# mhrice/RemFx

Hardware: AMD Instinct MI355X
Metric: audio-seconds/sec fwd+bwd (whole job) (higher is better)
Workload: dtype bf16 (fp32 accumulate); 1 GPU; Hybrid Demucs (cfg/model/demucs.yaml) train step, +exp=chorus_aug model=demucs; clips_per_gpu=64, global_batch=64, clip_samples=262144, parallelism=dp1, rccl_ranks=0, ranks=1, streams=4

## Files before the change

### include/remfx_hip.h

```cpp
#ifndef REMFX_HIP_H
#define REMFX_HIP_H

#include <stdint.h>

#ifdef __cplusplus
extern "C" {
#endif

#define RFX_ABI_VERSION 1

enum rfx_act {
  RFX_ACT_NONE = 0,
  RFX_ACT_RELU = 1,
  RFX_ACT_GELU = 2,
  RFX_ACT_TANH = 3,
  RFX_ACT_PRELU = 4,
  RFX_ACT_LEAKY = 5,
  RFX_ACT_SIGMOID = 6
};

typedef struct rfx_ktab_entry {
  int32_t off;
  int32_t da;
  int32_t db;
// ... 255 lines not shown
                       const float* sums, float w_sc, float w_lm, const float* gup, float* gxc, void* stream);
int64_t rfx_stft_pair_loss_ws(const rfx_stft_desc* d);
int rfx_stft_pair_loss(const rfx_stft_desc* d, const float* x, const float* y, const float* window, float eps, double* ws, float* sums,
                       float* xspec, float* ymag, void* stream);
int rfx_stft_loss_grad_m(const float* xc, const float* ymag, int32_t R, int64_t n, float eps, const float* sums, float w_sc,
                         float w_lm, const float* gup, float* gxc, void* stream);
int rfx_fft_synthesis_lossgrad(const rfx_stft_desc* d, const float* xspec, const float* ymag, const float* sums, float w_sc,
                               float w_lm, float eps, const float* gup, const float* window, float* ws, float* out, void* stream);
int rfx_l1_grad(const float* a, const float* b, int64_t n, float w, const float* gup, float* g, void* stream);
#define RFX_SISDR_SLOTS 128
int rfx_sisdr_sums(const float* x, const float* t, int32_t R, int64_t L, int64_t x_rs, int64_t t_rs,
                   double* ws, double* sums, void* stream);
int rfx_sisdr_finish(const double* sums, int32_t R, int64_t L, int32_t zero_mean, double eps, float* out, void* stream);
int rfx_mrstft_combine(const float* const* sums, const int64_t* n, int32_t nres, int32_t R, int32_t per_example_sc, float* out,
                       void* stream);

int rfx_zero(void* p, int64_t nbytes, void* stream);
#define RFX_SUMSQ_SLOTS 4096
int rfx_sumsq(const float* g, int64_t n, double* ws, double* out, void* stream);
int rfx_clip_coef(const double* sumsq, float max_norm, float pre, float* coef, float* norm_out, void* stream);
int rfx_adamw_step(float* p, const float* g, float* m, float* v, int64_t n, float lr, float b1, float b2,
                   float eps, float wd, int32_t step, const float* gscale, void* stream);

typedef struct rfx_cl_tensor {
  void* p;
  int64_t ns, as;
  int32_t bs, c0;
} rfx_cl_tensor;

enum rfx_cl_epi {
  RFX_CL_STORE = 0,
  RFX_CL_GELU = 1,
  RFX_CL_GLU = 2,
  RFX_CL_DGELU = 3,
  RFX_CL_STORE_CM = 5,
  RFX_CL_DGLU = 4
};

typedef struct rfx_cl_conv_desc {
  rfx_cl_tensor in;
  int32_t N, IA, IB, OA, OB, SA;
  int32_t NTR, NCH, NTC, KS;
  int32_t da0, da_step;
  int32_t db0, db_step;
  int32_t wrapb;
  const void* apack;
  int32_t M, BM;
  int32_t mode;
  int32_t G, g_off, OAo, Co;
  const float* bias;
  const float* rowadd;
  rfx_cl_tensor out0, out1, aux0, res;
  void* cm_out;
  int64_t cm_ns, cm_cs, cm_as;
  int32_t cm_fold;
} rfx_cl_conv_desc;
int rfx_cl_conv(const rfx_cl_conv_desc* d, void* stream);
int rfx_cl_pack(const float* src, const int32_t* idx, int64_t n, void* dst, void* stream);
int rfx_cl_from_cm(const void* src, int32_t src_bf16, int64_t s_ns, int64_t s_cs, int64_t s_as, int32_t N, int32_t C, int32_t A,
                   int32_t B, const rfx_cl_tensor* dst, const rfx_cl_tensor* res, const rfx_cl_tensor* aux, int32_t mode, void* stream);
int rfx_cl_to_cm(const rfx_cl_tensor* src, int32_t N, int32_t C, int32_t A, int32_t B, void* dst, int32_t dst_bf16, int64_t d_ns,
                 int64_t d_cs, int64_t d_as, const void* aux16, void* stream);
int rfx_cl_im2col_s4(const float* src, int64_t s_ns, int64_t s_cs, int64_t s_as, int32_t N, int32_t Cs, int32_t IA, int32_t IB, int32_t OA,
                     int32_t OB, int32_t along_b, void* dst, void* stream);
int rfx_cl_im2col_fm(const float* src, const float* coef_a, const float* coef_b, int32_t N, int32_t F, int32_t bins, void* dst, void* stream);
int rfx_fm_cm_affine(const float* in, float* out, const float* coef_a, const float* coef_b, int32_t N, int32_t bins, int32_t F, int32_t to_fm,
                     void* stream);
int rfx_cl_dgelu(const void* g, const void* z, void* out, int64_t n, void* stream);
int rfx_cl_dglu(const void* g, const void* zab, void* out, int64_t npos, int32_t C, void* stream);

typedef struct rfx_cl_wgrad_desc {
  rfx_cl_tensor p, q;
  int32_t N, OA, IA, B;
  int32_t SA, da0, NTR;
  int32_t NTC, db0, db_step;
  int32_t M, Cq, CW;
  int32_t RW, WK;
  int32_t S, ahead, bias;
  int32_t PW;
  float* ws;
} rfx_cl_wgrad_desc;
int64_t rfx_cl_wgrad_ws_floats(const rfx_cl_wgrad_desc* d);
int rfx_cl_wgrad(const rfx_cl_wgrad_desc* d, void* stream);
int rfx_cl_wgrad_reduce(const float* ws, const int32_t* map, int64_t nmap, int32_t S, int32_t DT, int32_t RW, int32_t WK, float* dw,
                        int64_t wn, float* db, int32_t accumulate, void* stream);

typedef struct rfx_cl_dconv_desc {
  const void* x;
  const void* gy;
  void* y;
  void* a; void* hpre; float* stats;
  void* dz; void* dh; float* partial;
  const void* w1p; const void* w2p; const void* w2dp; const void* w1dp;
  const float *b1, *g1w, *g1b, *b2, *g2w, *g2b, *scale;
  int32_t S, C, H, dil, grid, x_or_gy_ok;
  float eps;
  int32_t TPS;
  float* tsum; float* sums;
  float* pg_dst[5];
} rfx_cl_dconv_desc;
int rfx_cl_dconv_ok(int32_t C, int32_t H, int32_t T, int32_t backward);
int rfx_cl_dconv_fwd(const rfx_cl_dconv_desc* d, void* stream);
int rfx_cl_dconv_bwd(const rfx_cl_dconv_desc* d, float* pgrad, void* stream);

int rfx_cl_rowsum(const rfx_cl_tensor* x, int32_t N, int32_t A, int32_t B, int32_t C, int32_t G, float scale, float* partial, float* out,
                  int32_t accumulate, void* stream);

int rfx_abi_version(void);
int rfx_gemm_pick_r(int32_t M, int32_t K);

#ifdef __cplusplus
}
#endif
#endif
```

### remfx_amd/_lib.py

```python
import ctypes as C
import glob
import os
import subprocess

_HERE = os.path.dirname(os.path.abspath(__file__))
_ROOT = os.path.dirname(_HERE)
CSRC = os.path.join(_HERE, "csrc")
INCLUDE = os.path.join(_ROOT, "include")
LIBDIR = os.path.join(_HERE, "_C")
LIBPATH = os.environ.get("RFX_LIBPATH_DEV") or os.path.join(LIBDIR, "libremfx_hip.so")

HIPCC_FLAGS = ["--offload-arch=gfx950", "-O3", "-std=c++17", "-fPIC", "-ffp-contract=fast",
               "-I" + INCLUDE, "-I" + CSRC]


def sources():
    return sorted(glob.glob(os.path.join(CSRC, "*.hip")))


def _stale():
    if not os.path.exists(LIBPATH):
        return True
    t = os.path.getmtime(LIBPATH)
    deps = sources() + glob.glob(os.path.join(CSRC, "*.h")) + glob.glob(os.path.join(INCLUDE, "*.h"))
# ... 118 lines not shown
    "rfx_norm_bwd_work_floats": [_I32, _I32, _I32, _I32],
    "rfx_batchnorm_stat_slots": [_I32, _I32],
    "rfx_groupnorm_fwd": [_P, _P, _P, _I32, _I32, _I32, _I32, C.c_float, _I32, _P, _P, _P, _I32, _P, _P, _P, _P],
    "rfx_groupnorm_bwd": [_P, _P, _P, _P, _P, _P, _I32, _I32, _I32, _I32, _I32, _P, _P, _P, _P, _P, _P, _P],
    "rfx_groupnorm_fwd_x16": [_P, _P, _P, _I32, _I32, _I32, _I32, C.c_float, _I32, _P, _P, _P, _I32, _P, _P, _P, _P],
    "rfx_groupnorm_bwd_x16": [_P, _P, _P, _P, _P, _P, _I32, _I32, _I32, _I32, _I32, _P, _P, _P, _P, _P, _P, _P],
    "rfx_batchnorm_fwd": [_P, _P, _P, _I32, _I32, _I32, C.c_float, _I32, _I32, _P, _P, _P, _P, _P],
    "rfx_batchnorm_bwd": [_P, _P, _P, _P, _P, _P, _I32, _I32, _I32, _I32, _P, _P, _P, _P, _P],
    "rfx_avgpool2d_fwd": [_P, _P, _I64, _I32, _I32, _I32, _I32, _P],
    "rfx_avgpool2d_bwd": [_P, _P, _I64, _I32, _I32, _I32, _I32, _P],
    "rfx_cplx_slots": [_I32, _I64],
    "rfx_cplx_moments": [_P, _I32, _I32, _I64, _P, _P, _P],
    "rfx_cplx_moments_bwd": [_P, _P, _I32, _I32, _I64, _P, _P],
    "rfx_cplx_coef_fwd": [_P, C.c_double, _P, _P, _P, _P, _P, _P, C.c_float, _I32, _P, _P, _P, _P, _P, _P, _P, C.c_float, _P],
    "rfx_cplx_coef_bwd": [_P, C.c_double, _P, _P, _P, _P, _P, _P, C.c_float, _I32, _P, _P, _P, _P],
    "rfx_cplx_affine_act_fwd": [_P, _P, _I32, _I32, _I64, C.c_float, _P, _I64, _I64, _P],
    "rfx_cplx_affine_act_bwd": [_P, _P, _P, _I64, _I64, _I32, _I32, _I64, C.c_float, _P, _P, _P, _P],
    "rfx_bound_mask_fwd": [_P, _P, _P, _I32, _I64, _I64, _I64, _I64, _P],
    "rfx_bound_mask_bwd": [_P, _P, _P, _P, _I32, _I64, _I64, _I64, _I64, _I64, _P],
    "rfx_phase_mask_fwd": [_P, _P, _P, _I64, _P],
    "rfx_phase_mask_bwd": [_P, _P, _P, _I64, _P],
    "rfx_glu_fwd": [_P, _P, _I64, _I64, _I64, _P],
    "rfx_glu_bwd": [_P, _P, _P, _I64, _I64, _I64, _P],
    "rfx_glu_bwd_bf16": [_P, _P, _P, _I64, _I64, _I64, _P],
    "rfx_act_fwd": [_P, _P, _I64, _I32, _P],
    "rfx_act_bwd": [_P, _P, _P, _I64, _I32, _P],
    "rfx_act_add_fwd": [_P, _P, _P, _I64, _I32, _P],
    "rfx_act_rows": [_P, _I64, _I64, _I64, _P, _I64, _I64, _I64, _P, _I64, _I64, _I64, _I32, _I32, _I32, _I32, _I32, _P],
    "rfx_act_rows16": [_P, _I64, _I64, _I64, _P, _I64, _I64, _I64, _P, _I64, _I64, _I64, _I32, _I32, _I32, _I32, _I32, _P],
    "rfx_mul": [_P, _P, _P, _I64, _P],
    "rfx_prelu_fwd": [_P, _P, _P, _I64, _I64, _I64, _P],
    "rfx_prelu_bwd": [_P, _P, _P, _P, _P, _P, _I64, _I64, _I64, _P],
    "rfx_l1_sum": [_P, _P, _I64, _P, C.c_float, _P, _P],
    "rfx_add_bcast": [_P, _P, _P, _I64, _I32, _I32, _I32, _I64, _I64, _I64, _I64, C.c_float, _P],
    "rfx_localstate_fwd": [_P, _P, _P, _P, _I32, _I32, _I32, _I32, _I32, _P, _P, _P],
    "rfx_localstate_bwd": [_P, _P, _P, _P, _P, _P, _I32, _I32, _I32, _I32, _I32, _P, _P, _P, _P, _P],
    "rfx_dconv_layer_ok": [_I32, _I32, _I32],
    "rfx_dconv_layer_bwd_rows": [_I32],
    "rfx_dconv_layer_bwd": [_P, _P, _P, _I32, _I32, _I32, _I32, _P, _P, _P, _P, _P, _P, _P, _P, _P, C.c_float, _P, _P, _P, _P, _P],
    "rfx_dconv_layer_fwd": [_P, _P, _I32, _I32, _I32, _I32, _P, _P, _P, _P, _P, _P, _P, _P, _P, C.c_float, _P, _P, _P, _P, _P],
    "rfx_fx_distortion": [_P, _P, _I32, _I64, _P, _P],
    "rfx_fx_delay": [_P, _P, _I32, _I64, _P, _P, _P, _P],
    "rfx_fx_chorus": [_P, _P, _I32, _I64, C.c_float, _P, _P, _P, _P, _P, _P],
    "rfx_fx_compressor": [_P, _P, _P, _I32, _I64, _P, _P, _P, _P, _P],
    "rfx_fx_reverb": [_P, _P, _I32, _I64, _I32, _P, _P, _P, _P, _P],
    "rfx_fx_loudness": [_P, _I32, _I64, _I32, _I32, _I32, _I32, C.c_double, _P, C.c_float, _P, _P, _P, _P],
    "rfx_fx_scale": [_P, _P, _I32, _I64, _P, _P],
    "rfx_fx_loudness_joint": [_P, _I32, _I32, _I64, _I32, _I32, _I32, _I32, C.c_double, _P, C.c_float, _P, _P, _P, _P],
    "rfx_fx_limiter": [_P, _P, _P, _I32, _I64, _P, _P],
    "rfx_fx_eq": [_P, _P, _I32, _I64, _I32, _I32, _P, _P],
    "rfx_fx_widener": [_P, _P, _I32, _I64, _P, _P, _P],
    "rfx_fx_volume": [_P, _I32, _I64, _I32, _P, _P, _P, _P],
    "rfx_fx_phaser_ws_floats": [_I32, _I64],
    "rfx_fx_phaser": [_P, _P, _P, _I32, _I64, C.c_float, _P, _P, _P, _P, _P, _P],
    "rfx_localstate_gen_fwd": [_P, _P, _P, _P, _I32, _I32, _I32, _I32, _I32, _P, _P, _P],
    "rfx_localstate_gen_bwd": [_P, _P, _P, _P, _P, _P, _P, _I32, _I32, _I32, _I32, _I32, _P, _P, _P, _P, _P],
    "rfx_mha_fwd": [_P, _P, _P, _I32, _I32, _I32, _I32, _P, _P, _P],
    "rfx_mha_bwd": [_P, _P, _P, _P, _P, _P, _I32, _I32, _I32, _I32, _P, _P, _P, _P],
    "rfx_localstate_mfma_ok": [_I32, _I32, _I32, _I32, _I32],
    "rfx_localstate_mfma_fwd": [_P, _P, _P, _P, _I32, _I32, _I32, _I32, _I32, _P, _P],
    "rfx_localstate_mfma_bwd": [_P, _P, _P, _P, _P, _I32, _I32, _I32, _I32, _I32, _P, _P, _P, _P, _P, _P],
    "rfx_blstm_frames": [_P, _P, _P, _I32, _I32, _I32, _I32, _I32, _I32, _I32, _P],
    "rfx_span_mask": [_P, _I32, _I32, _I32, _P, _P, _P, _P, _P],
    "rfx_dropout": [_P, _P, _I64, C.c_float, C.c_uint64, _P],
    "rfx_row_moments_slots": [_I64],
    "rfx_row_moments": [_P, _I32, _I64, _P, _P, _P, C.c_float, _P, _P, _P],
    "rfx_row_affine": [_P, _P, _P, _P, _I32, _I64, _P],
    "rfx_lstm_pack_bytes": [_I32],
    "rfx_lstm_pack": [_P, _I32, _P, _P],
    "rfx_lstm_cat_params": [_P, _P, _P, _P, _P, _P, _I32, _I32, _P, _P, _P],
    "rfx_lstm_grad_scatter": [_P, _P, _I32, _I32, _P, _P, _P, _P, _P, _P, _P],
    "rfx_lstm_local": [_I32, _I32, _I32, _I32],
    "rfx_lstm_pack_local": [_P, _I32, _P, _P],
    "rfx_lstm_ws_bytes": [_I32],
    "rfx_lstm_fwd": [_P, _P, _I32, _I32, _I32, _P, _P, _P, _P, _I32, _P],
    "rfx_lstm_bwd": [_P, _P, _P, _P, _I32, _I32, _I32, _P, _P, _I32, _P],
    "rfx_lstm_set_local": [_I32, _I32],
    "rfx_channel_sum_ws": [_P, _I32, _I32, _I32, _I32, _I64, _I64, _I64, _I64],
    "rfx_channel_sum": [_P, _I32, _I32, _I32, _I32, _I64, _I64, _I64, _I64, _P, _P, _P],
    "rfx_cl_conv": [C.POINTER(ClConvDesc), _P],
    "rfx_cl_pack": [_P, _P, _I64, _P, _P],
    "rfx_cl_wgrad_ws_floats": [_P],
    "rfx_cl_wgrad": [_P, _P],
    "rfx_cl_wgrad_reduce": [_P, _P, _I64, _I32, _I32, _I32, _I32, _P, _I64, _P, _I32, _P],
    "rfx_cl_from_cm": [_P, _I32, _I64, _I64, _I64, _I32, _I32, _I32, _I32, C.POINTER(ClTensor), C.POINTER(ClTensor), C.POINTER(ClTensor),
                       _I32, _P],
    "rfx_cl_rowsum": [C.POINTER(ClTensor), _I32, _I32, _I32, _I32, _I32, C.c_float, _P, _P, _I32, _P],
    "rfx_cl_to_cm": [C.POINTER(ClTensor), _I32, _I32, _I32, _I32, _P, _I32, _I64, _I64, _I64, _P, _P],
    "rfx_cl_dgelu": [_P, _P, _P, _I64, _P],
    "rfx_cl_dglu": [_P, _P, _P, _I64, _I32, _P],
    "rfx_cl_im2col_s4": [_P, _I64, _I64, _I64, _I32, _I32, _I32, _I32, _I32, _I32, _I32, _P, _P],
    "rfx_cl_im2col_fm": [_P, _P, _P, _I32, _I32, _I32, _P, _P],
    "rfx_fm_cm_affine": [_P, _P, _P, _P, _I32, _I32, _I32, _I32, _P],
    "rfx_cl_dconv_ok": [_I32, _I32, _I32, _I32],
    "rfx_cl_dconv_fwd": [_P, _P],
    "rfx_cl_dconv_bwd": [_P, _P, _P],
}

_RET64 = {"rfx_cl_wgrad_ws_floats", "rfx_cplx_slots", "rfx_norm_bwd_work_floats", "rfx_stft_pair_loss_ws", "rfx_channel_sum_ws", "rfx_fft_synthesis_ws",
          "rfx_fx_phaser_ws_floats"}
_lib = None


def lib():
    global _lib
    if _lib is not None:
        return _lib
    import torch
    if not os.path.exists(LIBPATH):
        raise RuntimeError(
            f"{LIBPATH} not found: run `python -c 'import __graft_entry__ as g; g.build()'` "
            "(hipcc --offload-arch=gfx950).  remfx_amd has no CPU fallback.")
    L = C.CDLL(LIBPATH)
    for name, argtypes in SIGNATURES.items():
        fn = getattr(L, name)
        fn.argtypes = argtypes
        fn.restype = C.c_int64 if name in _RET64 else C.c_int
    if L.rfx_abi_version() != 1:
        raise RuntimeError("libremfx_hip ABI version mismatch")
    _lib = L
    return L


def check(rc, what):
    if rc != 0:
        raise RuntimeError(f"{what} failed with code {rc}")
```

### remfx_amd/clast.py

```python
import ctypes as C
import os as _os

import numpy as np
import torch

from . import _lib, ops
from ._lib import ClConvDesc, ClTensor, ClWgradDesc, check

EPI = {"store": 0, "gelu": 1, "glu": 2, "dgelu": 3, "dglu": 4, "store_cm": 5}


def _stream():
    return C.c_void_p(ops.raw_stream())


def cl_tensor(t, c0=0):
    ct = ClTensor()
    if t is None:
        return ct
    if t.dtype != torch.bfloat16 or t.dim() != 4 or t.stride(3) != 1 or not t.is_cuda:
        raise ValueError(f"channels-last operand must be a 4-D bf16 GPU tensor with dense channels (got {t.dtype}, {tuple(t.shape)}, {t.stride()})")
    ct.p = t.data_ptr()
    ct.ns, ct.as_, ct.bs, ct.c0 = t.stride(0), t.stride(1), t.stride(2), c0
    return ct
# ... 229 lines not shown
    N, Cs, IA, IB = x.shape
    if x.dtype != torch.float32 or x.stride(3) != 1:
        x = x.float().contiguous()
    out = empty(N, OA, OB, 16, x.device)
    check(_lib.lib().rfx_cl_im2col_s4(C.c_void_p(x.data_ptr()), x.stride(0), x.stride(1), x.stride(2), N, Cs, IA, IB, OA, OB, int(along_b),
                                      C.c_void_p(out.data_ptr()), _stream()), "rfx_cl_im2col_s4")
    return out


def im2col_fm(spec, a, b):
    N, F, bins, two = spec.shape
    if two != 2 or spec.dtype != torch.float32 or not spec.is_contiguous() or bins % 4:
        raise ValueError("im2col_fm: contiguous (N, frames, bins, 2) fp32 with bins % 4 == 0")
    out = empty(N, bins // 4, F, 16, spec.device)
    check(_lib.lib().rfx_cl_im2col_fm(C.c_void_p(spec.data_ptr()), C.c_void_p(a.data_ptr()), C.c_void_p(b.data_ptr()), N, F, bins,
                                      C.c_void_p(out.data_ptr()), _stream()), "rfx_cl_im2col_fm")
    return out


def form_head(Cout, Cs):
    def widx(m, r, t, ch):
        k, c = ch // Cs, ch % Cs
        return np.where(k < 8, (m * Cs + c) * 8 + np.minimum(k, 7), -1)
    return ConvForm(Cout, 16, 1, 1, 0, 0, 0, 0, 1, widx, KS=1)


def wform_head(Cout, Cs):
    def widx(m, r, t, c):
        return (m * Cs + c % Cs) * 8 + c // Cs
    return WgradForm(Cout, 8 * Cs, 1, 1, 1, 0, 0, 0, widx, Cout * Cs * 8)


def form_tail_tr(Cc, Cs):
    def widx(m, r, t, ch):
        psi, co = m // Cs, m % Cs
        return (ch * Cs + co) * 8 + psi + 4 * (1 - r)
    return ConvForm(4 * Cs, Cc, 2, 1, -1, 1, 0, 0, 1, widx, G=4, g_off=-2, Co=Cs)


def form_tail_dgrad(Cc, Cs):
    def widx(m, r, t, ch):
        k, co = ch // Cs, ch % Cs
        return np.where(k < 8, (m * Cs + co) * 8 + np.minimum(k, 7), -1)
    return ConvForm(Cc, 16, 1, 1, 0, 0, 0, 0, 1, widx, KS=1)


def wform_tail(Cc, Cs):
    def widx(m, r, t, c):
        return (m * Cs + c % Cs) * 8 + c // Cs
    return WgradForm(Cc, 8 * Cs, 1, 1, 1, 0, 0, 0, widx, Cc * Cs * 8, bias=False)


CLW_SPLITS = int(_os.environ.get("RFX_CLW_SPLITS", "256"))


class WgradForm:

    LDS_MAX = 160 * 1024

    def __init__(self, M, Cq, NTR, NTC, SA, da0, db0, db_step, widx, wn, bias=True):
        self.M, self.Cq, self.NTR, self.NTC, self.SA, self.da0, self.db0, self.db_step = M, Cq, NTR, NTC, SA, da0, db0, db_step
        self.wn, self.bias = wn, bias
        self.RW = 3 if M > 64 else 2
        T = NTR * NTC
        nb = 1 if bias else 0
        best = None
        for CW in (96, 80, 64, 48, 32, 16):
            if CW > -(-Cq // 16) * 16:
                continue
            tiles = -(-(T * CW // 16) // 2) + nb
            if tiles > 16:
                continue
            ctn = -(-Cq // CW)
            cost = (ctn, ctn * CW - Cq)
            if best is None or cost < best[0]:
                best = (cost, CW, tiles)
        if best is None:
            raise ValueError(f"channels-last weight gradient: no tiling for {T} taps x {Cq} channels")
        _, self.CW, tiles = best
        self.WK = 1 if tiles > 8 else (2 if tiles > 4 else 4)
        self.WC = 8 // self.WK
        self.MTn, self.CTn = -(-M // (32 * self.RW)), -(-Cq // self.CW)
        self.DT = self.MTn * self.CTn
        hb = max(abs(db0 + t * db_step) for t in range(NTC))
        self.ahead = None
        for PW, amin in (((128, 2), (64, 1)) if _os.environ.get("RFX_CLW_PW", "128") == "128" else ((64, 1),)):
            NP = PW // 16 * self.RW
            NQ = -(-((PW + 2 * hb) * self.CW * 2) // 1024)
            PPW = -(-(NP + SA * NQ) // 8)
            if PPW > 6 or (PW // 16) % self.WK:
                continue
            for ahead in (4, 3, 2, 1):
                R = -(-(NTR + ahead * SA) // SA) * SA
                if ahead >= amin and (ahead + 1) * NP * 1024 + R * NQ * 1024 <= self.LDS_MAX and (ahead - 1) * PPW <= 24:
                    self.ahead, self.PW = ahead, PW
                    break
            if self.ahead is not None:
                break
        if self.ahead is None:
            raise ValueError("channels-last weight gradient: tile does not fit LDS")
        self.map = self._build_map(widx)
        self._dev = {}

    def _build_map(self, widx):
        RW, NT, WC = self.RW, 2, self.WC
        NCG = self.CW // 16
        HN = self.NTR * self.NTC * NCG
        bias_tile = -(-HN // 2)
        shape = (self.MTn, self.CTn, WC, RW, NT, 16, 64)
        mt, ct, cw, i, t, r, lane = np.meshgrid(*[np.arange(s, dtype=np.int64) for s in shape], indexing="ij", sparse=True)
        m = mt * 32 * RW + 32 * i + (r & 3) + 8 * (r >> 2) + 4 * (lane >> 5)
        l31 = lane & 31
        tile = cw * NT + t
        hh = 2 * tile + (l31 >> 4)
        cgl, tt = hh % NCG, hh // NCG
        tc, tr = tt % self.NTC, tt // self.NTC
        c = ct * self.CW + cgl * 16 + (l31 & 15)
        ok = (hh < HN) & (m < self.M) & (c < self.Cq)
        idx = widx(np.minimum(m, self.M - 1), np.minimum(tr, self.NTR - 1), tc, np.minimum(c, self.Cq - 1))
        out = np.where(np.broadcast_to(ok, shape), np.broadcast_to(idx, shape), -1)
        if self.bias:
            isb = (tile == bias_tile) & (l31 == 0) & (ct == 0) & (m < self.M)
            out = np.where(np.broadcast_to(isb, shape), np.broadcast_to(self.wn + m, shape), out)
        flat = out.reshape(-1)
        used = flat[flat >= 0]
        assert used.size == np.unique(used).size, "weight-gradient map: a destination is written twice"
        return np.ascontiguousarray(flat.astype(np.int32))

    def splits(self, steps):
        S = max(1, min(steps, -(-CLW_SPLITS // self.DT)))
        sps = -(-steps // S)
        return -(-steps // sps)


def _dev_map(form, device):
    key = str(device)
    v = form._dev.get(key)
    if v is None:
        v = torch.from_numpy(form.map).to(device)
        form._dev[key] = v
    return v


def wgrad(form, p, q, N, OA, IA, B, dw, db=None, accumulate=False, p_c0=0, q_c0=0):
    if form.bias and db is None:
        raise ValueError("this weight-gradient form carries the bias gradient: pass db")
    d = ClWgradDesc()
    d.p, d.q = cl_tensor(p, p_c0), cl_tensor(q, q_c0)
    d.N, d.OA, d.IA, d.B = N, OA, IA, B
    d.SA, d.da0, d.NTR, d.NTC, d.db0, d.db_step = form.SA, form.da0, form.NTR, form.NTC, form.db0, form.db_step
    d.M, d.Cq, d.CW, d.RW, d.WK = form.M, form.Cq, form.CW, form.RW, form.WK
    PW = form.PW if B % form.PW == 0 else 64
    d.PW = PW
    d.S = form.splits(N * (B // PW) * OA)
    d.ahead, d.bias = min(form.ahead, int(_os.environ.get("RFX_CLW_AHEAD", "99"))), int(form.bias)
    L = _lib.lib()
    nws = L.rfx_cl_wgrad_ws_floats(C.byref(d))
    if nws <= 0:
        raise RuntimeError("rfx_cl_wgrad: geometry rejected")
    ws = torch.empty(nws, device=p.device, dtype=torch.float32)
    d.ws = ws.data_ptr()
    check(L.rfx_cl_wgrad(C.byref(d), _stream()), "rfx_cl_wgrad")
    mp = _dev_map(form, p.device)
    check(L.rfx_cl_wgrad_reduce(C.c_void_p(ws.data_ptr()), C.c_void_p(mp.data_ptr()), mp.numel(), d.S, form.DT, form.RW, form.WK,
                                C.c_void_p(dw.data_ptr()), form.wn, C.c_void_p(db.data_ptr()) if db is not None else None,
                                int(accumulate), _stream()), "rfx_cl_wgrad_reduce")


def wform_conv(Cout, Cin, KA, KB):
    def widx(m, r, t, c):
        return ((m * Cin + c) * KA + r) * KB + t
    return WgradForm(Cout, Cin, KA, KB, 1, -(KA // 2), -(KB // 2), 1, widx, Cout * Cin * KA * KB)


def wform_conv_s4(Cout, Cin):
    def widx(m, r, t, c):
        return (m * Cin + c) * 8 + r
    return WgradForm(Cout, Cin, 8, 1, 4, -2, 0, 0, widx, Cout * Cin * 8)


def wform_convtr_s4(Cin, Cout):
    def widx(m, r, t, c):
        return (m * Cout + c) * 8 + r
    return WgradForm(Cin, Cout, 8, 1, 4, -2, 0, 0, widx, Cin * Cout * 8, bias=False)

# ... 16 lines not shown
```

### remfx_amd/csrc/cl_wgrad.hip

```cpp
#include "cl_common.h"

#ifndef RFX_CLW_DBG_BUILD
#define RFX_CLW_DBG_BUILD 0
#endif
#define CLW_DBG RFX_CLW_DBG_BUILD
#include <stdlib.h>

struct ClWgK {
  rfx_cl_wgrad_desc d;
  int32_t nbq, MTn, CTn, DT, spx;
  int32_t total, sps;
  int32_t NP, NQ, TP, PPW;
  int32_t PSLOT, QROWB, QROWP, R, PD, PRE, HB;
  int32_t HN, NCG, bias_tile;
  uint32_t p_bytes, q_bytes;
};

#define CL_WG_MAXP 6

__device__ __forceinline__ void clw_wait_vm(int n) {
  switch (n) {
    case 0: CL_VMCNT(0); break;   case 1: CL_VMCNT(1); break;   case 2: CL_VMCNT(2); break;   case 3: CL_VMCNT(3); break;
    case 4: CL_VMCNT(4); break;   case 5: CL_VMCNT(5); break;   case 6: CL_VMCNT(6); break;   case 7: CL_VMCNT(7); break;
    case 8: CL_VMCNT(8); break;   case 9: CL_VMCNT(9); break;   case 10: CL_VMCNT(10); break; case 11: CL_VMCNT(11); break;
    case 12: CL_VMCNT(12); break; case 13: CL_VMCNT(13); break; case 14: CL_VMCNT(14); break; case 15: CL_VMCNT(15); break;
    case 16: CL_VMCNT(16); break; case 17: CL_VMCNT(17); break; case 18: CL_VMCNT(18); break; case 19: CL_VMCNT(19); break;
    case 20: CL_VMCNT(20); break; case 21: CL_VMCNT(21); break; case 22: CL_VMCNT(22); break; case 23: CL_VMCNT(23); break;
    default: CL_VMCNT(24); break;
  }
}

typedef short clw_s16x4 __attribute__((ext_vector_type(4)));
typedef short clw_s16x8 __attribute__((ext_vector_type(8)));
__device__ __forceinline__ cl_bf16x8 clw_frag(const unsigned char* p, int step4) {
  const clw_s16x4 lo = __builtin_amdgcn_ds_read_tr16_b64_v4i16((__attribute__((address_space(3))) clw_s16x4*)(p));
  const clw_s16x4 hi = __builtin_amdgcn_ds_read_tr16_b64_v4i16((__attribute__((address_space(3))) clw_s16x4*)(p + step4));
  const clw_s16x8 v = {lo[0], lo[1], lo[2], lo[3], hi[0], hi[1], hi[2], hi[3]};
  return __builtin_bit_cast(cl_bf16x8, v);
}

struct ClwIt {
  int n, bq, oa, pre;
};

template <int RW, int WK, int PW>
__global__ __launch_bounds__(512, 2) void cl_wgrad_kernel(const ClWgK g) {
  constexpr int NT = 2, WC = 8 / WK, KSW = (PW / 16) / WK;
  constexpr int PROWB = 64 * RW;
  extern __shared__ __attribute__((aligned(16))) unsigned char clw_smem[];
  const rfx_cl_wgrad_desc& d = g.d;
  const int tid = threadIdx.x;
  const int wave = __builtin_amdgcn_readfirstlane(tid >> 6), lane = tid & 63;
  const int kq = wave / WC, cw = wave % WC;
  const int bid = blockIdx.x, xcd = bid & 7, qx = bid >> 3;
  const bool grouped = d.S >= 8;
  const int dt = grouped ? qx % g.DT : bid % g.DT, split = grouped ? xcd * g.spx + qx / g.DT : bid / g.DT;
  if (split >= d.S) return;
  const int mt = dt / g.CTn, ct = dt - mt * g.CTn;
  const int tau0 = split * g.sps;
  const int tau1 = min(tau0 + g.sps, g.total);
  const int OA = d.OA;

  unsigned char* const pbase_lds = clw_smem;
  unsigned char* const qbase_lds = clw_smem + g.PD * g.PSLOT;

  int32_t rel[CL_WG_MAXP], bpos[CL_WG_MAXP];
  int lds_off[CL_WG_MAXP], prow[CL_WG_MAXP];
#pragma unroll
  for (int i = 0; i < CL_WG_MAXP; ++i) {
    int e = wave + 8 * i;
    e = e < g.TP ? e : g.TP - 1;
    if (e < g.NP) {
      prow[i] = -1;
      lds_off[i] = e * 1024;
      const int o = e * 1024 + lane * 16;
      const int pos = o / PROWB, cb = o - pos * PROWB;
      const bool ok = pos < PW && (mt * 32 * RW + (cb >> 1)) < d.M;
      rel[i] = ok ? (int32_t)((pos * d.p.bs + d.p.c0 + mt * 32 * RW) * 2 + cb) : (int32_t)CL_OOB;
      bpos[i] = 0;
    } else {
      const int qe = e - g.NP;
      const int rr = qe / g.NQ, qi = qe - rr * g.NQ;
      prow[i] = rr;
      lds_off[i] = rr * g.QROWB + qi * 1024;
      const int o = qi * 1024 + lane * 16;
      const int pos = o / g.QROWP, cb = o - pos * g.QROWP;
      const bool ok = pos < PW + 2 * g.HB && (ct * d.CW + (cb >> 1)) < d.Cq;
      rel[i] = ok ? (int32_t)(((pos - g.HB) * d.q.bs + d.q.c0 + ct * d.CW) * 2 + cb) : (int32_t)CL_OOB;
      bpos[i] = ok ? pos - g.HB : 0x40000000;
    }
  }

  const int gq = lane >> 4, i16 = lane & 15;
  const int rowhalf = gq & 1, khalf = gq >> 1, s_e = i16 >> 2, q4 = i16 & 3;
  const uint32_t a0 = (uint32_t)((8 * khalf + s_e) * PROWB + rowhalf * 32 + q4 * 8);
  int rtap[NT];
  uint32_t bconst[NT];
#pragma unroll
  for (int t = 0; t < NT; ++t) {
    int hh = 2 * (cw * NT + t) + rowhalf;
    hh = hh < g.HN ? hh : 0;
    const int cgl = hh % g.NCG, tt = hh / g.NCG;
    const int tc = tt % d.NTC;
    rtap[t] = tt / d.NTC;
    bconst[t] = (uint32_t)((g.HB + d.db0 + tc * d.db_step + 8 * khalf + s_e) * g.QROWP + cgl * 32 + q4 * 8);
  }
  const bool ones_wave = d.bias && g.bias_tile >= 0 && (g.bias_tile / NT) == cw;
  const int ones_t = g.bias_tile % NT;

  f32x16 acc[RW][NT];
#pragma unroll
  for (int i = 0; i < RW; ++i)
#pragma unroll
    for (int t = 0; t < NT; ++t)
#pragma unroll
      for (int r = 0; r < 16; ++r) acc[i][t][r] = 0.f;

  const int col0 = tau0 / OA;
  const int ncols = (tau1 - 1) / OA - col0 + 1;
  const int L = (tau1 - tau0) + g.PRE * ncols;
  ClwIt it_i = {col0 / g.nbq, col0 % g.nbq, tau0 - col0 * OA - g.PRE, g.PRE}, it_c = it_i;
  auto advance = [&](ClwIt& it) {
    ++it.oa;
    if (it.pre > 0) --it.pre;
    if (it.oa == OA) {
      it.oa = -g.PRE; it.pre = g.PRE;
      if (++it.bq == g.nbq) { it.bq = 0; ++it.n; }
    }
  };
  int rs_n = it_i.n;
  cl_i32x4 rs_p = cl_rsrc_words(reinterpret_cast<const uint16_t*>(d.p.p) + (int64_t)rs_n * d.p.ns, g.p_bytes);
  cl_i32x4 rs_q = cl_rsrc_words(reinterpret_cast<const uint16_t*>(d.q.p) + (int64_t)rs_n * d.q.ns, g.q_bytes);
  int iu = 0, wp = 0, ps_i = 0;
  auto issue_next = [&]() {
    if (CLW_DBG & 1) { advance(it_i); ++iu; return; }
    const int b0 = it_i.bq * PW;
    const bool real = it_i.pre == 0;
    if (it_i.n != rs_n) {
      rs_n = it_i.n;
      rs_p = cl_rsrc_words(reinterpret_cast<const uint16_t*>(d.p.p) + (int64_t)rs_n * d.p.ns, g.p_bytes);
      rs_q = cl_rsrc_words(reinterpret_cast<const uint16_t*>(d.q.p) + (int64_t)rs_n * d.q.ns, g.q_bytes);
    }
    const int32_t pb = (int32_t)(((int64_t)it_i.oa * d.p.as + (int64_t)b0 * d.p.bs) * 2);
    const int ia0 = it_i.oa * d.SA + d.da0 + d.NTR - d.SA;
#pragma unroll
    for (int i = 0; i < CL_WG_MAXP; ++i) {
      if (i < g.PPW) {
        if (prow[i] < 0) {
          const uint32_t vo = real ? (uint32_t)(rel[i] + pb) : CL_OOB;
          cl_glds16_quiet(rs_p, pbase_lds + ps_i * g.PSLOT + lds_off[i], vo);
        } else {
          const int ia = ia0 + prow[i];
          const bool rok = (unsigned)ia < (unsigned)d.IA;
          const int32_t qb = (int32_t)(((int64_t)ia * d.q.as + (int64_t)b0 * d.q.bs) * 2);
          const uint32_t vo = (rok && (unsigned)(b0 + bpos[i]) < (unsigned)d.B) ? (uint32_t)(rel[i] + qb) : CL_OOB;
          cl_glds16_quiet(rs_q, qbase_lds + wp * g.QROWB + lds_off[i], vo);
        }
      }
    }
    wp += d.SA;
    wp = wp >= g.R ? wp - g.R : wp;
    ps_i = ps_i + 1 == g.PD ? 0 : ps_i + 1;
    advance(it_i);
    ++iu;
  };

  int cpm = (d.SA - d.NTR + 2 * g.R) % g.R;
  int ps_c = 0;
  const int ahead = g.PD - 1;
  for (int i = 0; i < ahead; ++i)
    if (iu < L) issue_next();
  const bool late = wave >= 4 && !(CLW_DBG & 16);
  auto frags = [&](int ks, const unsigned char* pb, const unsigned char* const (&qb)[NT], cl_bf16x8 (&af)[RW], cl_bf16x8 (&bf)[NT], int i) {
#pragma unroll
    for (int r = 0; r < RW; ++r)
      af[r] = (CLW_DBG & 2) ? __builtin_bit_cast(cl_bf16x8, make_uint4(lane, r, ks, i)) : clw_frag(pb + ks * 16 * PROWB + r * 64, 4 * PROWB);
#pragma unroll
    for (int t = 0; t < NT; ++t) {
      if (ones_wave && t == ones_t) {
        const clw_s16x8 one = {0x3f80, 0x3f80, 0x3f80, 0x3f80, 0x3f80, 0x3f80, 0x3f80, 0x3f80};
        bf[t] = __builtin_bit_cast(cl_bf16x8, one);
      } else {
        bf[t] = (CLW_DBG & 2) ? __builtin_bit_cast(cl_bf16x8, make_uint4(lane, t, ks, i)) : clw_frag(qb[t] + ks * 16 * g.QROWP, 4 * g.QROWP);
      }
    }
  };
  for (int i = 0; i < L; ++i) {
    const int left = L - 1 - i;
    clw_wait_vm((left < ahead - 1 ? left : ahead - 1) * g.PPW);
    if (!(CLW_DBG & 8)) __builtin_amdgcn_s_barrier();
    __builtin_amdgcn_sched_barrier(0);
    if (!late && iu < L) issue_next();
    __builtin_amdgcn_sched_barrier(0);
    if (it_c.pre == 0 && !(CLW_DBG & 4)) {
      const unsigned char* pb = pbase_lds + ps_c * g.PSLOT + a0;
      const unsigned char* qb[NT];
#pragma unroll
      for (int t = 0; t < NT; ++t) {
        int sl = cpm + rtap[t];
        sl = sl >= g.R ? sl - g.R : sl;
        qb[t] = qbase_lds + sl * g.QROWB + bconst[t];
      }
      cl_bf16x8 af[2][RW], bf[2][NT];
      frags(kq, pb, qb, af[0], bf[0], i);
#pragma unroll
      for (int ksi = 0; ksi < KSW; ++ksi) {
        if (ksi + 1 < KSW) frags(kq + (ksi + 1) * WK, pb, qb, af[(ksi + 1) & 1], bf[(ksi + 1) & 1], i);
#pragma unroll
        for (int r = 0; r < RW; ++r)
#pragma unroll
          for (int t = 0; t < NT; ++t) acc[r][t] = __builtin_amdgcn_mfma_f32_32x32x16_bf16(af[ksi & 1][r], bf[ksi & 1][t], acc[r][t], 0, 0, 0);
      }
    }
    __builtin_amdgcn_sched_barrier(0);
    if (late && iu < L) issue_next();
    cpm += d.SA;
    cpm = cpm >= g.R ? cpm - g.R : cpm;
    ps_c = ps_c + 1 == g.PD ? 0 : ps_c + 1;
    advance(it_c);
  }

  float* wsp = d.ws + ((size_t)((size_t)split * g.DT + dt) * 8 + wave) * (RW * NT * 16 * 64) + lane;
#pragma unroll
  for (int r = 0; r < RW; ++r)
#pragma unroll
    for (int t = 0; t < NT; ++t)
#pragma unroll
      for (int e = 0; e < 16; ++e) wsp[((r * NT + t) * 16 + e) * 64] = acc[r][t][e];
}

static int clw_geometry(const rfx_cl_wgrad_desc& d, ClWgK& k) {
  if (d.N <= 0 || d.OA <= 0 || d.IA <= 0 || d.B <= 0 || (d.PW != 64 && d.PW != 128) || d.B % d.PW) return -1;
  if (d.NTR < 1 || d.NTR > 16 || d.NTC < 1 || d.NTC > 9 || d.SA < 1 || d.SA > d.NTR) return -1;
  if (d.M <= 0 || d.Cq <= 0 || d.CW < 16 || d.CW % 16 || d.CW > 128) return -1;
  if ((d.RW != 2 && d.RW != 3) || (d.WK != 1 && d.WK != 2 && d.WK != 4)) return -1;
  if (d.PW == 64 && d.WK == 4 && false) return -1;
  if (d.p.bs % 8 || d.p.c0 % 8 || d.q.bs % 8 || d.q.c0 % 8 || d.S < 1 || d.ahead < 1) return -1;
  int hb = 0;
  for (int t = 0; t < d.NTC; ++t) {
    const int v = d.db0 + t * d.db_step;
    hb = v < 0 ? (-v > hb ? -v : hb) : (v > hb ? v : hb);
  }
  if (hb > 8) return -1;
  k.d = d;
  k.HB = hb;
  k.nbq = d.B / d.PW;
  k.MTn = (d.M + 32 * d.RW - 1) / (32 * d.RW);
  k.CTn = (d.Cq + d.CW - 1) / d.CW;
  k.DT = k.MTn * k.CTn;
  k.spx = (d.S + 7) / 8;
  const int64_t total = (int64_t)d.N * k.nbq * d.OA;
  if (total >= 0x7fffffffLL) return -1;
  k.total = (int)total;
  k.sps = (int)((total + d.S - 1) / d.S);
  if ((total + k.sps - 1) / k.sps != d.S) return -1;
  k.NCG = d.CW / 16;
  k.HN = d.NTR * d.NTC * k.NCG;
  const int WC = 8 / d.WK, tiles = (k.HN + 1) / 2;
  if (tiles > WC * 2) return -1;
  k.bias_tile = d.bias ? tiles : -1;
  if (d.bias && tiles + 1 > WC * 2) return -1;
  k.NP = (d.PW * 64 * d.RW + 1023) / 1024;
  k.QROWP = d.CW * 2;
  k.NQ = ((d.PW + 2 * hb) * k.QROWP + 1023) / 1024;
  k.TP = k.NP + d.SA * k.NQ;
  k.PPW = (k.TP + 7) / 8;
  if (k.PPW > CL_WG_MAXP) return -1;
  k.PSLOT = k.NP * 1024;
  k.QROWB = k.NQ * 1024;
  k.PRE = (d.NTR - d.SA + d.SA - 1) / d.SA;
  k.PD = d.ahead + 1;
  k.R = ((d.NTR + d.ahead * d.SA + d.SA - 1) / d.SA) * d.SA;
  if ((k.PD - 2) * k.PPW > 24 && k.PD > 2) return -1;
  const int64_t pb = ((int64_t)(d.OA - 1) * d.p.as + (int64_t)d.B * d.p.bs) * 2;
  const int64_t qb = ((int64_t)(d.IA - 1) * d.q.as + (int64_t)d.B * d.q.bs) * 2;
  if (pb <= 0 || qb <= 0 || pb >= 0x7fffffffLL || qb >= 0x7fffffffLL) return -1;
  k.p_bytes = (uint32_t)pb;
  k.q_bytes = (uint32_t)qb;
  return 0;
}

template <int RW, int WK, int PW>
static int clw_launch1(const ClWgK& k, int lds, hipStream_t s) {
  static int attr_lds = 0;
  if (lds > attr_lds) {
    if (hipFuncSetAttribute(reinterpret_cast<const void*>(&cl_wgrad_kernel<RW, WK, PW>), hipFuncAttributeMaxDynamicSharedMemorySize, lds) !=
        hipSuccess)
      return -3;
    attr_lds = lds;
  }
  hipLaunchKernelGGL((cl_wgrad_kernel<RW, WK, PW>), dim3((unsigned)(k.d.S >= 8 ? 8 * k.spx * k.DT : k.d.S * k.DT)), dim3(512), lds, s, k);
  RFX_CHECK_LAUNCH();
  return 0;
}
template <int RW, int WK>
static int clw_launch(const ClWgK& k, int lds, hipStream_t s) {
  return k.d.PW == 128 ? clw_launch1<RW, WK, 128>(k, lds, s) : clw_launch1<RW, WK, 64>(k, lds, s);
}

extern "C" int64_t rfx_cl_wgrad_ws_floats(const rfx_cl_wgrad_desc* dp) {
  ClWgK k;
  if (!dp || clw_geometry(*dp, k)) return -1;
  return (int64_t)dp->S * k.DT * 8 * dp->RW * 2 * 1024;
}

extern "C" int rfx_cl_wgrad(const rfx_cl_wgrad_desc* dp, void* stream) {
  if (!dp || !dp->p.p || !dp->q.p || !dp->ws) return -1;
  ClWgK k;
  if (clw_geometry(*dp, k)) return -1;
  const int lds = k.PD * k.PSLOT + k.R * k.QROWB;
  if (lds > 160 * 1024) return -1;
  hipStream_t s = (hipStream_t)stream;
  if (dp->RW == 3) {
    if (dp->WK == 1) return clw_launch<3, 1>(k, lds, s);
    if (dp->WK == 2) return clw_launch<3, 2>(k, lds, s);
    return clw_launch<3, 4>(k, lds, s);
  }
  if (dp->WK == 1) return clw_launch<2, 1>(k, lds, s);
  if (dp->WK == 2) return clw_launch<2, 2>(k, lds, s);
  return clw_launch<2, 4>(k, lds, s);
}

__global__ __launch_bounds__(256) void cl_wgrad_reduce_kernel(const float* __restrict__ ws, const int32_t* __restrict__ map, int64_t nmap,
                                                              int S, int DT, int WC, int WK, int per_wave, float* __restrict__ dw,
                                                              int64_t wn, float* __restrict__ db, int accumulate) {
  __shared__ float part[4][64];
  const int l = threadIdx.x & 63, sg = threadIdx.x >> 6;
  const int64_t e = (int64_t)blockIdx.x * 64 + l;
  const int32_t dst = e < nmap ? map[e] : -1;
  float sum = 0.f;
  if (dst >= 0) {
    const int64_t inner = e % per_wave;
    const int64_t dc = e / per_wave;
    const int cw = (int)(dc % WC);
    const int64_t dt = dc / WC;
    const int nsrc = S * WK;
    const int per = (nsrc + 3) / 4;
    const int i0 = sg * per, i1 = min(i0 + per, nsrc);
    const int64_t sstride = (int64_t)DT * 8 * per_wave;
    const float* base = ws + dt * 8 * per_wave + (int64_t)cw * per_wave + inner;
    auto src = [&](int i) { return base[(int64_t)(i / WK) * sstride + (int64_t)(i % WK) * WC * per_wave]; };
    int i = i0;
    for (; i + 8 <= i1; i += 8) {
      float v[8];
#pragma unroll
      for (int u = 0; u < 8; ++u) v[u] = src(i + u);
#pragma unroll
      for (int u = 0; u < 8; ++u) sum += v[u];
    }
    for (; i < i1; ++i) sum += src(i);
  }
  part[sg][l] = sum;
  __syncthreads();
  if (sg == 0 && dst >= 0) {
    const float tot = ((part[0][l] + part[1][l]) + part[2][l]) + part[3][l];
    float* o = dst >= wn ? db + (dst - wn) : dw + dst;
    *o = accumulate ? *o + tot : tot;
  }
}

extern "C" int rfx_cl_wgrad_reduce(const float* ws, const int32_t* map, int64_t nmap, int32_t S, int32_t DT, int32_t RW, int32_t WK,
                                   float* dw, int64_t wn, float* db, int32_t accumulate, void* stream) {
  if (!ws || !map || !dw || nmap <= 0 || S < 1 || DT < 1 || (RW != 2 && RW != 3) || (WK != 1 && WK != 2 && WK != 4)) return -1;
  const int WC = 8 / WK, per_wave = RW * 2 * 16 * 64;
  if (nmap != (int64_t)DT * WC * per_wave) return -1;
  hipLaunchKernelGGL(cl_wgrad_reduce_kernel, dim3((unsigned)((nmap + 63) / 64)), dim3(256), 0, (hipStream_t)stream, ws, map, nmap, S,
                     DT, WC, WK, per_wave, dw, wn, db, accumulate);
  RFX_CHECK_LAUNCH();
  return 0;
}
```

Baseline: 3718 audio-seconds/sec.

## Swizzle LDS layout in channels-last wgrad kernel to reduce bank conflicts

Adds an XOR-64 swizzle for the P and Q staging tiles in LDS and a permuted K-stride layout when the channel-group count is odd. It also pads Q rows and picks the filler half-tile that minimises bank-conflict degree on the host. Fragment addresses and global-to-LDS source mappings now go through shared layout helpers, and Python tile selection asks the native plan function instead of duplicating the arithmetic. The aim is to cut LDS bank conflicts in the MFMA fragment loads of the weight-gradient kernel, at the cost of extra address arithmetic and slightly more LDS from row padding.

```diff
diff --git a/include/remfx_hip.h b/include/remfx_hip.h
--- a/include/remfx_hip.h
+++ b/include/remfx_hip.h
@@ -361,6 +361,8 @@
 } rfx_cl_wgrad_desc;
 int64_t rfx_cl_wgrad_ws_floats(const rfx_cl_wgrad_desc* d);
 int rfx_cl_wgrad(const rfx_cl_wgrad_desc* d, void* stream);
+int rfx_cl_wgrad_plan(const rfx_cl_wgrad_desc* d, int32_t* out);
+int rfx_cl_wgrad_lds_probe(const rfx_cl_wgrad_desc* d, int32_t dense, int32_t what, int32_t a, int32_t b, int32_t c, int32_t* out);
 int rfx_cl_wgrad_reduce(const float* ws, const int32_t* map, int64_t nmap, int32_t S, int32_t DT, int32_t RW, int32_t WK, float* dw,
                         int64_t wn, float* db, int32_t accumulate, void* stream);
 
diff --git a/remfx_amd/_lib.py b/remfx_amd/_lib.py
--- a/remfx_amd/_lib.py
+++ b/remfx_amd/_lib.py
@@ -224,6 +224,8 @@
     "rfx_cl_pack": [_P, _P, _I64, _P, _P],
     "rfx_cl_wgrad_ws_floats": [_P],
     "rfx_cl_wgrad": [_P, _P],
+    "rfx_cl_wgrad_plan": [_P, _P],
+    "rfx_cl_wgrad_lds_probe": [_P, _I32, _I32, _I32, _I32, _I32, _P],
     "rfx_cl_wgrad_reduce": [_P, _P, _I64, _I32, _I32, _I32, _I32, _P, _I64, _P, _I32, _P],
     "rfx_cl_from_cm": [_P, _I32, _I64, _I64, _I64, _I32, _I32, _I32, _I32, C.POINTER(ClTensor), C.POINTER(ClTensor), C.POINTER(ClTensor),
                        _I32, _P],
diff --git a/remfx_amd/clast.py b/remfx_amd/clast.py
--- a/remfx_amd/clast.py
+++ b/remfx_amd/clast.py
@@ -335,17 +335,13 @@
         self.WC = 8 // self.WK
         self.MTn, self.CTn = -(-M // (32 * self.RW)), -(-Cq // self.CW)
         self.DT = self.MTn * self.CTn
-        hb = max(abs(db0 + t * db_step) for t in range(NTC))
         self.ahead = None
         for PW, amin in (((128, 2), (64, 1)) if _os.environ.get("RFX_CLW_PW", "128") == "128" else ((64, 1),)):
-            NP = PW // 16 * self.RW
-            NQ = -(-((PW + 2 * hb) * self.CW * 2) // 1024)
-            PPW = -(-(NP + SA * NQ) // 8)
-            if PPW > 6 or (PW // 16) % self.WK:
+            if (PW // 16) % self.WK:
                 continue
             for ahead in (4, 3, 2, 1):
-                R = -(-(NTR + ahead * SA) // SA) * SA
-                if ahead >= amin and (ahead + 1) * NP * 1024 + R * NQ * 1024 <= self.LDS_MAX and (ahead - 1) * PPW <= 24:
+                plan = self.plan(PW, ahead)
+                if ahead >= amin and plan is not None and plan["fits"]:
                     self.ahead, self.PW = ahead, PW
                     break
             if self.ahead is not None:
@@ -354,6 +350,26 @@
             raise ValueError("channels-last weight gradient: tile does not fit LDS")
         self.map = self._build_map(widx)
         self._dev = {}
+
+    PLAN_FIELDS = ("NP", "NQ", "TP", "PPW", "PSLOT", "QROWB", "QROWP", "R", "PD", "PRE", "HB", "lds", "KSTR", "HN", "HFILL", "fits")
+
+    def desc(self, PW, ahead, N=1, OA=1, B=None):
+        d = ClWgradDesc()
+        d.N, d.OA, d.IA, d.B = N, OA, (OA - 1) * self.SA + self.NTR, B or PW
+        d.SA, d.da0, d.NTR, d.NTC, d.db0, d.db_step = self.SA, self.da0, self.NTR, self.NTC, self.db0, self.db_step
+        d.M, d.Cq, d.CW, d.RW, d.WK = self.M, self.Cq, self.CW, self.RW, self.WK
+        d.PW, d.S, d.ahead, d.bias = PW, 1, ahead, int(self.bias)
+        for t, ch in ((d.p, self.M), (d.q, self.Cq)):
+            t.bs = -(-ch // 8) * 8
+            t.as_ = d.B * t.bs
+            t.ns = d.IA * t.as_
+        return d
+
+    def plan(self, PW, ahead):
+        out = (C.c_int32 * 16)()
+        if _lib.lib().rfx_cl_wgrad_plan(C.byref(self.desc(PW, ahead)), out):
+            return None
+        return dict(zip(self.PLAN_FIELDS, out))
 
     def _build_map(self, widx):
         RW, NT, WC = self.RW, 2, self.WC
diff --git a/remfx_amd/csrc/cl_wgrad.hip b/remfx_amd/csrc/cl_wgrad.hip
--- a/remfx_amd/csrc/cl_wgrad.hip
+++ b/remfx_amd/csrc/cl_wgrad.hip
@@ -13,8 +13,50 @@
   int32_t NP, NQ, TP, PPW;
   int32_t PSLOT, QROWB, QROWP, R, PD, PRE, HB;
   int32_t HN, NCG, bias_tile;
+  int32_t KSTR, X64P, X64Q, QHI, HFILL;
   uint32_t p_bytes, q_bytes;
 };
+
+struct ClwLay {
+  int32_t PW, HB, PROWB, QROWP, KSTR, X64P, X64Q;
+};
+__host__ __device__ inline int clw_kpos(const ClwLay& l, int ks, int kb, int hl, int q) {
+  return 16 * ks + 8 * kb + (l.KSTR == 2 ? hl + 2 * q : 4 * hl + q);
+}
+__host__ __device__ inline int clw_p_slot(const ClwLay& l, int pos) {
+  return l.KSTR == 2 ? (pos & ~7) | ((pos & 1) << 2) | ((pos >> 1) & 3) : pos;
+}
+__host__ __device__ inline int clw_p_unslot(const ClwLay& l, int slot) {
+  return l.KSTR == 2 ? (slot & ~7) | ((slot & 3) << 1) | ((slot >> 2) & 1) : slot;
+}
+__host__ __device__ inline uint32_t clw_p_off(const ClwLay& l, int pos, int cb) {
+  const int sl = clw_p_slot(l, pos);
+  return (uint32_t)(sl * l.PROWB + (cb ^ ((l.X64P && (sl & 2)) ? 64 : 0)));
+}
+__host__ __device__ inline void clw_p_src(const ClwLay& l, int o, int& pos, int& cb) {
+  const int sl = o / l.PROWB;
+  pos = clw_p_unslot(l, sl);
+  cb = (o - sl * l.PROWB) ^ ((l.X64P && (sl & 2)) ? 64 : 0);
+}
+__host__ __device__ inline uint32_t clw_q_off(const ClwLay& l, int ip, int cb) {
+  return (uint32_t)(ip * l.QROWP + (cb ^ ((l.X64Q && (ip & 2)) ? 64 : 0)));
+}
+__host__ __device__ inline void clw_q_src(const ClwLay& l, int o, int& ip, int& cb) {
+  ip = o / l.QROWP;
+  cb = (o - ip * l.QROWP) ^ ((l.X64Q && (ip & 2)) ? 64 : 0);
+}
+__host__ __device__ inline uint32_t clw_frag_p(const ClwLay& l, int lane, int r) {
+  const int gq = lane >> 4, i16 = lane & 15;
+  return clw_p_off(l, clw_kpos(l, 0, gq >> 1, 0, i16 >> 2), r * 64 + (gq & 1) * 32 + (i16 & 3) * 8);
+}
+__host__ __device__ inline uint32_t clw_frag_q(const ClwLay& l, int lane, int cgl, int db) {
+  const int gq = lane >> 4, i16 = lane & 15;
+  return clw_q_off(l, l.HB + db + clw_kpos(l, 0, gq >> 1, 0, i16 >> 2), cgl * 32 + (i16 & 3) * 8);
+}
+__host__ __device__ inline int clw_q_hi(const ClwLay& l) { return (l.KSTR == 2 ? 1 : 4) * l.QROWP; }
+__host__ __device__ inline ClwLay clw_lay(const ClWgK& g) {
+  return ClwLay{g.d.PW, g.HB, 64 * g.d.RW, g.QROWP, g.KSTR, g.X64P, g.X64Q};
+}
 
 #define CL_WG_MAXP 6
 
@@ -64,6 +106,8 @@
   unsigned char* const pbase_lds = clw_smem;
   unsigned char* const qbase_lds = clw_smem + g.PD * g.PSLOT;
 
+  ClwLay lay = clw_lay(g);
+  lay.X64P = RW == 2;
   int32_t rel[CL_WG_MAXP], bpos[CL_WG_MAXP];
   int lds_off[CL_WG_MAXP], prow[CL_WG_MAXP];
 #pragma unroll
@@ -73,8 +117,8 @@
     if (e < g.NP) {
       prow[i] = -1;
       lds_off[i] = e * 1024;
-      const int o = e * 1024 + lane * 16;
-      const int pos = o / PROWB, cb = o - pos * PROWB;
+      int pos, cb;
+      clw_p_src(lay, e * 1024 + lane * 16, pos, cb);
       const bool ok = pos < PW && (mt * 32 * RW + (cb >> 1)) < d.M;
       rel[i] = ok ? (int32_t)((pos * d.p.bs + d.p.c0 + mt * 32 * RW) * 2 + cb) : (int32_t)CL_OOB;
       bpos[i] = 0;
@@ -83,27 +127,28 @@
       const int rr = qe / g.NQ, qi = qe - rr * g.NQ;
       prow[i] = rr;
       lds_off[i] = rr * g.QROWB + qi * 1024;
-      const int o = qi * 1024 + lane * 16;
-      const int pos = o / g.QROWP, cb = o - pos * g.QROWP;
+      int pos, cb;
+      clw_q_src(lay, qi * 1024 + lane * 16, pos, cb);
       const bool ok = pos < PW + 2 * g.HB && (ct * d.CW + (cb >> 1)) < d.Cq;
       rel[i] = ok ? (int32_t)(((pos - g.HB) * d.q.bs + d.q.c0 + ct * d.CW) * 2 + cb) : (int32_t)CL_OOB;
       bpos[i] = ok ? pos - g.HB : 0x40000000;
     }
   }
 
-  const int gq = lane >> 4, i16 = lane & 15;
-  const int rowhalf = gq & 1, khalf = gq >> 1, s_e = i16 >> 2, q4 = i16 & 3;
-  const uint32_t a0 = (uint32_t)((8 * khalf + s_e) * PROWB + rowhalf * 32 + q4 * 8);
+  const int rowhalf = (lane >> 4) & 1;
+  uint32_t pa[RW];
+#pragma unroll
+  for (int r = 0; r < RW; ++r) pa[r] = clw_frag_p(lay, lane, r);
   int rtap[NT];
   uint32_t bconst[NT];
 #pragma unroll
   for (int t = 0; t < NT; ++t) {
     int hh = 2 * (cw * NT + t) + rowhalf;
-    hh = hh < g.HN ? hh : 0;
+    hh = hh < g.HN ? hh : g.HFILL;
     const int cgl = hh % g.NCG, tt = hh / g.NCG;
     const int tc = tt % d.NTC;
     rtap[t] = tt / d.NTC;
-    bconst[t] = (uint32_t)((g.HB + d.db0 + tc * d.db_step + 8 * khalf + s_e) * g.QROWP + cgl * 32 + q4 * 8);
+    bconst[t] = clw_frag_q(lay, lane, cgl, d.db0 + tc * d.db_step);
   }
   const bool ones_wave = d.bias && g.bias_tile >= 0 && (g.bias_tile / NT) == cw;
   const int ones_t = g.bias_tile % NT;
@@ -174,14 +219,14 @@
   auto frags = [&](int ks, const unsigned char* pb, const unsigned char* const (&qb)[NT], cl_bf16x8 (&af)[RW], cl_bf16x8 (&bf)[NT], int i) {
 #pragma unroll
     for (int r = 0; r < RW; ++r)
-      af[r] = (CLW_DBG & 2) ? __builtin_bit_cast(cl_bf16x8, make_uint4(lane, r, ks, i)) : clw_frag(pb + ks * 16 * PROWB + r * 64, 4 * PROWB);
+      af[r] = (CLW_DBG & 2) ? __builtin_bit_cast(cl_bf16x8, make_uint4(lane, r, ks, i)) : clw_frag(pb + ks * 16 * PROWB + pa[r], 4 * PROWB);
 #pragma unroll
     for (int t = 0; t < NT; ++t) {
       if (ones_wave && t == ones_t) {
         const clw_s16x8 one = {0x3f80, 0x3f80, 0x3f80, 0x3f80, 0x3f80, 0x3f80, 0x3f80, 0x3f80};
         bf[t] = __builtin_bit_cast(cl_bf16x8, one);
       } else {
-        bf[t] = (CLW_DBG & 2) ? __builtin_bit_cast(cl_bf16x8, make_uint4(lane, t, ks, i)) : clw_frag(qb[t] + ks * 16 * g.QROWP, 4 * g.QROWP);
+        bf[t] = (CLW_DBG & 2) ? __builtin_bit_cast(cl_bf16x8, make_uint4(lane, t, ks, i)) : clw_frag(qb[t] + ks * 16 * g.QROWP, g.QHI);
       }
     }
   };
@@ -193,7 +238,7 @@
     if (!late && iu < L) issue_next();
     __builtin_amdgcn_sched_barrier(0);
     if (it_c.pre == 0 && !(CLW_DBG & 4)) {
-      const unsigned char* pb = pbase_lds + ps_c * g.PSLOT + a0;
+      const unsigned char* pb = pbase_lds + ps_c * g.PSLOT;
       const unsigned char* qb[NT];
 #pragma unroll
       for (int t = 0; t < NT; ++t) {
@@ -229,12 +274,40 @@
       for (int e = 0; e < 16; ++e) wsp[((r * NT + t) * 16 + e) * 64] = acc[r][t][e];
 }
 
+static void clw_half_addr(const ClwLay& l, const ClWgK& k, int hh, int lane, int& row, uint32_t& addr) {
+  const int cgl = hh % k.NCG, tt = hh / k.NCG;
+  row = tt / k.d.NTC;
+  addr = clw_frag_q(l, lane, cgl, k.d.db0 + (tt % k.d.NTC) * k.d.db_step);
+}
+static int clw_q_degree(const ClwLay& l, const ClWgK& k, int h0, int h1) {
+  int worst = 0;
+  for (int half = 0; half < 2; ++half)
+    for (int hl = 0; hl < 2; ++hl) {
+      uint32_t seen[64][4];
+      int n[64] = {0};
+      for (int i = 0; i < 32; ++i) {
+        const int lane = 32 * half + i;
+        int row;
+        uint32_t a;
+        clw_half_addr(l, k, (lane >> 4) & 1 ? h1 : h0, lane, row, a);
+        a += (uint32_t)(row * k.QROWB + hl * clw_q_hi(l));
+        for (int w = 0; w < 2; ++w) {
+          const uint32_t dw = a / 4 + w;
+          int j = 0;
+          while (j < n[dw % 64] && seen[dw % 64][j] != dw) ++j;
+          if (j == n[dw % 64] && j < 4) seen[dw % 64][n[dw % 64]++] = dw;
+        }
+      }
+      for (int b = 0; b < 64; ++b) worst = n[b] > worst ? n[b] : worst;
+    }
+  return worst;
+}
+
 static int clw_geometry(const rfx_cl_wgrad_desc& d, ClWgK& k) {
   if (d.N <= 0 || d.OA <= 0 || d.IA <= 0 || d.B <= 0 || (d.PW != 64 && d.PW != 128) || d.B % d.PW) return -1;
   if (d.NTR < 1 || d.NTR > 16 || d.NTC < 1 || d.NTC > 9 || d.SA < 1 || d.SA > d.NTR) return -1;
   if (d.M <= 0 || d.Cq <= 0 || d.CW < 16 || d.CW % 16 || d.CW > 128) return -1;
   if ((d.RW != 2 && d.RW != 3) || (d.WK != 1 && d.WK != 2 && d.WK != 4)) return -1;
-  if (d.PW == 64 && d.WK == 4 && false) return -1;
   if (d.p.bs % 8 || d.p.c0 % 8 || d.q.bs % 8 || d.q.c0 % 8 || d.S < 1 || d.ahead < 1) return -1;
   int hb = 0;
   for (int t = 0; t < d.NTC; ++t) {
@@ -262,16 +335,33 @@
   if (d.bias && tiles + 1 > WC * 2) return -1;
   k.NP = (d.PW * 64 * d.RW + 1023) / 1024;
   k.QROWP = d.CW * 2;
+  const bool odd = (k.NCG & 1) && k.NCG > 1;
+  k.KSTR = odd ? 2 : 1;
+  k.X64P = d.RW == 2;
+  k.X64Q = k.QROWP == 128;
+  const int rowpad = odd && d.NTR > 1 ? 32 : 0;
+  k.QHI = (k.KSTR == 2 ? 1 : 4) * k.QROWP;
   k.NQ = ((d.PW + 2 * hb) * k.QROWP + 1023) / 1024;
   k.TP = k.NP + d.SA * k.NQ;
   k.PPW = (k.TP + 7) / 8;
   if (k.PPW > CL_WG_MAXP) return -1;
   k.PSLOT = k.NP * 1024;
-  k.QROWB = k.NQ * 1024;
+  k.QROWB = k.NQ * 1024 + rowpad;
   k.PRE = (d.NTR - d.SA + d.SA - 1) / d.SA;
   k.PD = d.ahead + 1;
   k.R = ((d.NTR + d.ahead * d.SA + d.SA - 1) / d.SA) * d.SA;
+  if (rowpad && (k.R & 1)) k.R += d.SA;
+  if (rowpad && (k.R & 1)) return -1;
   if ((k.PD - 2) * k.PPW > 24 && k.PD > 2) return -1;
+  k.HFILL = 0;
+  if (k.HN & 1) {
+    const ClwLay l = clw_lay(k);
+    int best = 99;
+    for (int f = 0; f < k.HN; ++f) {
+      const int deg = clw_q_degree(l, k, k.HN - 1, f);
+      if (deg < best) { best = deg; k.HFILL = f; }
+    }
+  }
   const int64_t pb = ((int64_t)(d.OA - 1) * d.p.as + (int64_t)d.B * d.p.bs) * 2;
   const int64_t qb = ((int64_t)(d.IA - 1) * d.q.as + (int64_t)d.B * d.q.bs) * 2;
   if (pb <= 0 || qb <= 0 || pb >= 0x7fffffffLL || qb >= 0x7fffffffLL) return -1;
@@ -304,11 +394,65 @@
   return (int64_t)dp->S * k.DT * 8 * dp->RW * 2 * 1024;
 }
 
+static int clw_lds_bytes(const ClWgK& k) { return k.PD * k.PSLOT + k.R * k.QROWB; }
+
+extern "C" int rfx_cl_wgrad_plan(const rfx_cl_wgrad_desc* dp, int32_t* out) {
+  ClWgK k;
+  if (!dp || !out || clw_geometry(*dp, k)) return -1;
+  const int32_t v[16] = {k.NP, k.NQ, k.TP, k.PPW, k.PSLOT, k.QROWB, k.QROWP, k.R, k.PD, k.PRE, k.HB, clw_lds_bytes(k),
+                         k.KSTR, k.HN, k.HFILL, clw_lds_bytes(k) <= 160 * 1024};
+  for (int i = 0; i < 16; ++i) out[i] = v[i];
+  return 0;
+}
+
+extern "C" int rfx_cl_wgrad_lds_probe(const rfx_cl_wgrad_desc* dp, int32_t dense, int32_t what, int32_t a, int32_t b, int32_t c,
+                                      int32_t* out) {
+  ClWgK k;
+  if (!dp || !out || clw_geometry(*dp, k)) return -1;
+  if (dense) {
+    k.KSTR = 1; k.X64P = 0; k.X64Q = 0; k.QROWB = k.NQ * 1024; k.HFILL = 0;
+  }
+  const ClwLay l = clw_lay(k);
+  const int PW = dp->PW, gq = (a >> 4) & 3, i16 = a & 15;
+  int pos, cb;
+  if (what == 0 || what == 1) {
+    if (a < 0 || a >= (what ? k.NQ : k.NP) || b < 0 || b > 63) return -1;
+    const int o = a * 1024 + b * 16;
+    if (what == 0) clw_p_src(l, o, pos, cb); else clw_q_src(l, o, pos, cb);
+    out[0] = o;
+    out[1] = pos < (what ? PW + 2 * k.HB : PW) ? pos : -1;
+    out[2] = cb;
+    return 0;
+  }
+  if (a < 0 || a > 63 || c < 0 || c >= 2 * (PW / 16)) return -1;
+  const int ks = c >> 1, hl = c & 1, kp = clw_kpos(l, ks, gq >> 1, hl, i16 >> 2);
+  if (what == 2) {
+    if (b < 0 || b >= dp->RW) return -1;
+    out[0] = (int32_t)clw_frag_p(l, a, b) + ks * 16 * l.PROWB + hl * 4 * l.PROWB;
+    out[1] = kp;
+    out[2] = b * 64 + (gq & 1) * 32 + (i16 & 3) * 8;
+    return 0;
+  }
+  if (what == 3) {
+    int hh = b < k.HN ? b : k.HFILL, row;
+    if (b < 0) return -1;
+    uint32_t addr;
+    clw_half_addr(l, k, hh, a, row, addr);
+    const int tc = (hh / k.NCG) % dp->NTC;
+    out[0] = (int32_t)addr + row * k.QROWB + ks * 16 * k.QROWP + hl * clw_q_hi(l);
+    out[1] = k.HB + dp->db0 + tc * dp->db_step + kp;
+    out[2] = (hh % k.NCG) * 32 + (i16 & 3) * 8;
+    out[3] = row;
+    return 0;
+  }
+  return -1;
+}
+
 extern "C" int rfx_cl_wgrad(const rfx_cl_wgrad_desc* dp, void* stream) {
   if (!dp || !dp->p.p || !dp->q.p || !dp->ws) return -1;
   ClWgK k;
   if (clw_geometry(*dp, k)) return -1;
-  const int lds = k.PD * k.PSLOT + k.R * k.QROWB;
+  const int lds = clw_lds_bytes(k);
   if (lds > 160 * 1024) return -1;
   hipStream_t s = (hipStream_t)stream;
   if (dp->RW == 3) {
```

Result: no change. 3721 audio-seconds/sec (median of 6 runs) (+0.1%).
